# sangminwoo/Temporal-Span-Proposal-Network-VidVRD

Measured on AMD Instinct MI355X. Metric: tracklet-pairs/sec scored (N=32, T=150, D=2048), higher is better.
Workload: dtype f32

## Files before the change

### include/tspn_mi355x.h

```cpp
#ifndef TSPN_MI355X_H
#define TSPN_MI355X_H

#include <stddef.h>
#include <stdint.h>

#ifdef __cplusplus
extern "C" {
#endif

#define TSPN_ABI_VERSION 7

enum {
  TSPN_OK = 0,
  TSPN_EINVAL = -1,
  TSPN_EUNSUPPORTED = -2,
  TSPN_EWORKSPACE = -3,
  TSPN_ELAUNCH = -4,
  TSPN_EDEVICE = -5
};

#define TSPN_STATUS_WORDS 16
enum {
  TSPN_STATUS_FAULT = 0,
  TSPN_STATUS_FAULT_INFO = 1,
// ... 74 lines not shown
int tspn_conv3_f32(const float* x, int64_t B, int64_t Cin, int64_t T,
                   const float* packed, int64_t M, const float* bias, int relu,
                   float* y, void* stream);

int tspn_conv3_tc_f32(const float* x, int64_t B, int64_t T, int64_t Cin,
                      const float* packed, int64_t M, const float* bias, int relu,
                      float* y, void* stream);

int tspn_pack_conv3_wino63_frag_f32(const float* W, int64_t M, int64_t Cin, int64_t split, float* frag,
                                    void* stream);
size_t tspn_conv3_tc_wino63_workspace_bytes(int64_t B, int64_t T, int64_t Cin);
int tspn_conv3_tc_wino63_f32(const float* x, int64_t B, int64_t T, int64_t Cin, const float* frag,
                             int64_t M, const float* bias, int relu, float* y,
                             void* workspace, size_t workspace_bytes, void* stream);
int tspn_conv3_tc_wino63_set_piece_form(int form);

size_t tspn_pack_conv3_wino63_f16x3_elements(int64_t M, int64_t Cin, int64_t split);
int tspn_pack_conv3_wino63_f16x3(const float* W, int64_t M, int64_t Cin, int64_t split, int16_t* packed, void* stream);
size_t tspn_conv3_tc_wino63_f16x3_workspace_bytes(int64_t B, int64_t T, int64_t Cin, int64_t M);
int tspn_conv3_tc_wino63_f16x3(const float* x, int64_t B, int64_t T, int64_t Cin, const int16_t* packed,
                               int64_t M, const float* bias, int relu, float* y,
                               void* workspace, size_t workspace_bytes, void* stream);
int tspn_conv3_tc_wino63_f16x3_set_tail_split(int on);
int tspn_conv3_tc_wino63_f16x3_input_form(int64_t NT, int64_t T, int64_t Cin, int cus);
int tspn_conv3_tc_wino63_f16x3_set_input_form(int form);
int tspn_conv3_tc_wino63_f16x3_input(const float* x, int64_t B, int64_t T, int64_t Cin, int64_t M, void* split_input,
                                     size_t split_input_bytes, float* fbar, uint64_t* hot_slots, void* stream);


int tspn_heads_f32(int mode, const float* a, const float* b, int64_t lda,
                   const int64_t* ia, const int64_t* ib, int64_t idx_stride, const float* bias,
                   const float* Wh, const float* bh, int64_t H,
                   int64_t P, int64_t C, int64_t T, float* out, void* stream);

int tspn_heads_pairgrid_f32(const float* y, int64_t B, int64_t N, int64_t C, int64_t T,
                            const float* Wh, const float* bh, int64_t H, float* out,
                            void* stream);

size_t tspn_heads_pairgrid_f16x3_split_bytes(int64_t C, int64_t H);
int tspn_heads_pairgrid_f16x3_set_force_exact(int on);
int tspn_heads_pair_f16x3_set_diag_skip(int on);
int tspn_heads_pairgrid_f16x3(const float* y, int64_t ldt, int64_t B, int64_t N, int64_t C, int64_t T,
                              const float* Wh, const float* bh, int64_t H, void* split_buf, size_t split_bytes,
                              float* out, void* stream);

int tspn_temporal_mean_f32(const float* x, int64_t R, int64_t T, int64_t Cdim,
// ... 258 lines not shown
```

### temporal-span-proposal-network-vidvrd_amd/_abi.py

```python
import ctypes
import os
import re
import threading

HERE = os.path.dirname(os.path.abspath(__file__))
ROOT = os.path.dirname(HERE)
LIB_PATH = os.environ.get("TSPN_LIB_PATH") or os.path.join(HERE, "libtspn_mi355x.so")
HEADER_PATH = os.path.join(ROOT, "include", "tspn_mi355x.h")

ABI_VERSION = 7
TSPN_OK = 0
TSPN_EINVAL = -1
TSPN_EUNSUPPORTED = -2
TSPN_EWORKSPACE = -3
TSPN_ELAUNCH = -4
TSPN_EDEVICE = -5
STATUS_WORDS = 16
STATUS_FAULT, STATUS_FAULT_INFO, STATUS_CONV_ERR, STATUS_CONV_CHECKS = 0, 1, 2, 3
FAULT_HANDOVER = 1
CONV_CHECK_HOT_OFFSET, CONV_CHECK_SCRATCH_BYTES = 256, 256 + 256 * 64
GEOM_CHANNELS = 8
CONV_DIRECT, CONV_WINOGRAD63, CONV_WINOGRAD63_F16X3 = 0, 1, 2

_c_f32p = ctypes.c_void_p
# ... 102 lines not shown
                                               _vp, _vp]),
    "tspn_bottleneck_block_res_bf16": (_int, [_vp, _i64, _i64, _i64, _i64, _i64, _i64, _vp, _vp, _vp, _vp, _vp, _vp, _vp, _vp, _vp]),
    "tspn_bottleneck_tail_io_bf16": (_int, [_vp, _i64, _i64, _i64, _i64, _vp, _vp, _vp, _vp, _vp, _vp, _vp]),
    "tspn_bottleneck_tail_pipe_bf16": (_int, [_vp, _i64, _i64, _i64, _i64, _vp, _vp, _vp, _vp, _vp, _vp, _i64, _vp]),
    "tspn_bottleneck_tail_next_bf16": (_int, [_vp, _i64, _i64, _i64, _i64, _vp, _vp, _vp, _vp, _vp, _vp, _vp, _vp, _vp, _vp]),
    "tspn_stem_bf16_workspace_bytes": (_sz, [_i64, _i64, _i64]),
    "tspn_pack_stem_bf16": (_int, [_vp, _i64, _vp, _vp]),
    "tspn_stem_conv_bf16": (_int, [_vp, _i64, _i64, _i64, _vp, _i64, _vp, _vp, _sz, _vp, _vp]),
    "tspn_max_pool_nhwc_bf16": (_int, [_vp, _i64, _i64, _i64, _i64, _i64, _i64, _i64, _vp, _vp]),
    "tspn_stem_pool_bf16": (_int, [_vp, _i64, _i64, _i64, _vp, _i64, _vp, _vp, _sz, _vp, _vp]),
    "tspn_roi_align_nhwc_bf16": (_int, [_vp, _i64, _i64, _i64, _i64, _vp, _i64, _i64, ctypes.c_float, _int, _int,
                                        _int, _vp, _vp]),
    "tspn_roi_align_nhwc_f32_bf16out": (_int, [_vp, _i64, _i64, _i64, _i64, _vp, _i64, _i64, ctypes.c_float, _int, _int,
                                               _int, _vp, _vp]),
    "tspn_pack_conv3_wino63_frag_f32": (_int, [_vp, _i64, _i64, _i64, _vp, _vp]),
    "tspn_conv3_tc_wino63_workspace_bytes": (_sz, [_i64, _i64, _i64]),
    "tspn_conv3_tc_wino63_f32": (_int, [_vp, _i64, _i64, _i64, _vp, _i64, _vp, _int, _vp, _vp, _sz, _vp]),
    "tspn_conv3_tc_wino63_set_piece_form": (_int, [_int]),
    "tspn_pack_conv3_wino63_f16x3_elements": (_sz, [_i64, _i64, _i64]),
    "tspn_pack_conv3_wino63_f16x3": (_int, [_vp, _i64, _i64, _i64, _vp, _vp]),
    "tspn_conv3_tc_wino63_f16x3_workspace_bytes": (_sz, [_i64, _i64, _i64, _i64]),
    "tspn_conv3_tc_wino63_f16x3": (_int, [_vp, _i64, _i64, _i64, _vp, _i64, _vp, _int, _vp, _vp, _sz, _vp]),
    "tspn_conv3_tc_wino63_f16x3_set_tail_split": (_int, [_int]),
    "tspn_conv3_tc_wino63_f16x3_input_form": (_int, [_i64, _i64, _i64, _int]),
    "tspn_conv3_tc_wino63_f16x3_set_input_form": (_int, [_int]),
    "tspn_conv3_tc_wino63_f16x3_input": (_int, [_vp, _i64, _i64, _i64, _i64, _vp, _sz, _vp, _vp, _vp]),
    "tspn_span_predicate_workspace_bytes": (_sz, [_i64, _i64, _i64, _i64]),
    "tspn_span_predicate_f32": (_int, [_vp, _i64, _i64, _i64, _vp, _vp, _i64, _vp, _vp, _i64, _vp, _vp, _sz, _vp]),
    "tspn_decode_span_relations_workspace_bytes": (_sz, [_i64] * 8),
    "tspn_decode_span_relations_f32": (_int, [_vp, _i64, _i64, _i64, _i64, _vp, _i64, _vp, _vp, _vp, _i64, _vp, _vp, _i64,
                                              _vp, _i64, _i64, _i64, _vp, _vp, _vp, _vp, _vp, _vp, _vp, _sz, _vp]),
    "tspn_cast_bf16": (_int, [_vp, _i64, _vp, _vp]),
    "tspn_pack_conv3_bf16": (_int, [_vp, _i64, _i64, _i64, _vp, _vp]),
    "tspn_transpose_cast_bf16": (_int, [_vp, _i64, _i64, _i64, _vp, _vp]),
    "tspn_heads_dense_bf16": (_int, [_vp, _i64, _i64, _i64, _i64, _vp, _vp, _i64, _vp, _vp]),
    "tspn_temporal_encoder_heads_bf16": (_int, [_vp, _i64, _i64, _i64, _vp, _vp, _vp, _vp, _i64, _vp, _vp, _vp]),
    "tspn_pack_heads_bf16": (_int, [_vp, _i64, _i64, _vp, _vp]),
    "tspn_conv3_tc_bf16": (_int, [_vp, _i64, _i64, _i64, _vp, _i64, _vp, _vp, _i64, _vp]),
    "tspn_heads_pairgrid_bf16": (_int, [_vp, _i64, _i64, _i64, _i64, _i64, _vp, _vp, _i64, _vp, _vp]),
    "tspn_temporal_mean_bf16": (_int, [_vp, _i64, _i64, _i64, _vp, _vp]),
    "tspn_forward_fused_bf16_workspace_bytes": (_sz, [ctypes.POINTER(FusedBf16Desc)]),
    "tspn_forward_fused_bf16": (_int, [ctypes.POINTER(FusedBf16Desc), _vp]),
    "tspn_pair_plan_i32": (_int, [_vp, _i64, _i64, _i64, _vp, _vp, _vp, _vp, _vp, _vp, _vp]),
    "tspn_heads_pairlist_bf16_workspace_bytes": (_sz, [_i64, _i64, _i64]),
    "tspn_heads_pairlist_bf16": (_int, [_vp, _i64, _i64, _i64, _i64, _i64, _vp, _i64, _vp, _vp, _i64, _vp, _vp, _sz, _vp]),
    "tspn_forward_fused_bf16_pairs_workspace_bytes": (_sz, [ctypes.POINTER(FusedBf16Desc)]),
# ... 79 lines not shown
```

### temporal-span-proposal-network-vidvrd_amd/csrc/tspn_wino63.hip

```cpp
#include <algorithm>
#include <atomic>
#include <type_traits>

#include "tspn_common.h"
#include "tspn_device.h"
#include "tspn_wino63_input.h"

namespace {

using namespace tspn_dev;

constexpr int NW = 4;
constexpr int THREADS = 64 * NW;
constexpr int BM = 128;
constexpr int ST = 32;
constexpr int SWG = 64;
constexpr int KC = 8;
constexpr int NJ = 8;
constexpr int VROW = ST * 4;
constexpr int VCH = 2 * NJ * VROW;
constexpr int VHALF = 4 * VCH;
constexpr int VSS = 2 * VHALF;
constexpr int NVB = 2;
constexpr int NPIECE = 16;
// ... 393 lines not shown
    f32x4 V[2][8];
    transform(cg, V, false, xm);
#pragma unroll
    for (int j = 0; j < NJ; ++j) {
      f16x8 hi, lo;
#pragma unroll
      for (int i = 0; i < 8; ++i) {
        _Float16 h, l;
        wino63_split_f16(V[i >> 2][j][i & 3], ecol[j], h, l);
        hi[i] = h;
        lo[i] = l;
      }
      _Float16* dst = Vh + (((int64_t)j * 2 * ncg + cg) * nsp2 + S) * 8;
      *reinterpret_cast<f16x8*>(dst) = hi;
      *reinterpret_cast<f16x8*>(dst + (int64_t)ncg * nsp2 * 8) = lo;
    }
  }
}

#ifndef TSPN_WINO63_F16X3_STAGGER
#define TSPN_WINO63_F16X3_STAGGER 1
#endif
template <int WN, bool BUF>
__device__ __forceinline__ void wino63_f16x3_tile(
    char* smem_raw, const _Float16* __restrict__ Vh, const int* __restrict__ Ve, const int16_t* __restrict__ Wp,
    const float* __restrict__ bias, float* __restrict__ y, float* __restrict__ park, int Cin, int T, int M, int nq,
    int64_t nsext, int64_t nsp2, int tile_m, int tile_n, int tiles_n, int sub, int relu, int ldy, int vec2) {
  constexpr int MI = WN;
  constexpr int BN = 64 * WN;
  constexpr int NP = 16 + 4 * WN;
  constexpr int PW = (NP + 7) / 8;
  constexpr bool EVEN = NP % 8 == 0;
  constexpr bool STAGGER = TSPN_WINO63_F16X3_STAGGER && WN == 4;
  const int m0 = tile_m * F_BM;
  const int64_t S0 = (int64_t)tile_n * F_BN + sub * BN;

  const int tid = threadIdx.x;
  const int lane = tid & 63;
  const int wave = __builtin_amdgcn_readfirstlane(tid >> 6);
  const int wm = wave / WN, wn = wave % WN;
  const int li = lane & 31, kh = lane >> 5;
  const int ncg = Cin >> 3, nk = Cin >> 4;
  const int G = NJ * nk;

  const int p0 = wave * NP / 8;
  const int npw = EVEN ? PW : (wave + 1) * NP / 8 - p0;
  const int16_t* src[PW];
  unsigned voff[PW];
  int ldst[PW];
#pragma unroll
  for (int i = 0; i < PW; ++i) {
    const int p = min(p0 + i, NP - 1);
    int64_t el;
    if (p < 16) {
      const int region = p >> 3, cgi = (p >> 2) & 1, r = 64 * (p & 3) + lane;
      el = (((int64_t)region * ncg + cgi) * M + m0 + r) * 8;
      src[i] = Wp + el;
      ldst[i] = p * 1024;
    } else {
      const int v = p - 16;
      const int region = v / (2 * WN), cgi = (v / WN) & 1, r = 64 * (v % WN) + lane;
      el = (((int64_t)region * ncg + cgi) * nsp2 + S0 + r) * 8;
      src[i] = reinterpret_cast<const int16_t*>(Vh) + el;
      ldst[i] = (2 + region) * 8192 + cgi * 4096 + (v % WN) * 1024;
    }
    voff[i] = (unsigned)(el * 2);
  }
  int ik = 0, ist = 0;
  const char* wbase = reinterpret_cast<const char*>(Wp);
  const char* vbase = reinterpret_cast<const char*>(Vh);
  auto issue = [&]() {
    char* dst = smem_raw + ist * F_ST;
#pragma unroll
    for (int i = 0; i < PW; ++i)
      if (EVEN || i < npw) {
        if (BUF) bglds16(buffer_rsrc_unbounded(p0 + i < 16 ? wbase : vbase), voff[i], 0, dst + ldst[i]);
        else glds16(src[i], dst + ldst[i]);
      }
    ist = (ist + 1) & 3;
    const bool wrap = ++ik == nk;
    if (wrap) ik = 0;
    const int64_t dw = (int64_t)M * (wrap ? 32 * nk + 48 : 32), dv = nsp2 * (wrap ? 32 * nk + 32 : 32);
    if (BUF) {
      wbase += dw;
      vbase += dv;
    } else {
#pragma unroll
      for (int i = 0; i < PW; ++i) src[i] = reinterpret_cast<const int16_t*>(reinterpret_cast<const char*>(src[i]) + (p0 + i < 16 ? dw : dv));
    }
  };
  auto wait_stages = [&](auto ahead_tag) {
    constexpr int AHEAD = decltype(ahead_tag)::value;
    if (EVEN || npw == PW) wait_vmcnt<AHEAD * PW>(); else wait_vmcnt<AHEAD * (PW - 1)>();
  };

  f32x16 acc[MI][2];
#pragma unroll
  for (int mi = 0; mi < MI; ++mi)
#pragma unroll
    for (int ni = 0; ni < 2; ++ni)
#pragma unroll
      for (int e = 0; e < 16; ++e) acc[mi][ni][e] = 0.f;

  float* my_park = park + (int64_t)(tile_m * tiles_n + tile_n) * (F_PARK_PER_TILE / sizeof(float)) +
                   (int64_t)sub * (8 * MI) * F_THREADS * 4 + tid * 4;
  int* etab = reinterpret_cast<int*>(smem_raw + F_SMEM);
  auto unscale = [&](int j) {
    if (tid < F_BM)
      etab[tid] = reinterpret_cast<const int*>(Wp + (int64_t)j * (2 * ncg + 1) * M * 8 + (int64_t)2 * ncg * M * 8)[(int64_t)(m0 + tid) * 4];
    else if (tid - F_BM < BN)
      etab[tid] = Ve[(int64_t)j * nsp2 + S0 + tid - F_BM];
    __syncthreads();
    int ec[2];
#pragma unroll
    for (int ni = 0; ni < 2; ++ni) ec[ni] = etab[F_BM + wn * 64 + ni * 32 + li];
#pragma unroll
    for (int mi = 0; mi < MI; ++mi)
// ... 33 lines not shown
#pragma unroll
      for (int mi = 0; mi < MI; ++mi)
#pragma unroll
        for (int ni = 0; ni < 2; ++ni)
#pragma unroll
          for (int eq = 0; eq < 4; ++eq) {
            const f32x4 v = {acc[mi][ni][4 * eq], acc[mi][ni][4 * eq + 1], acc[mi][ni][4 * eq + 2], acc[mi][ni][4 * eq + 3]};
            *reinterpret_cast<f32x4*>(my_park + ((int64_t)j * 32 + (mi * 2 + ni) * 4 + eq) * F_THREADS * 4) = v;
#pragma unroll
            for (int e = 0; e < 4; ++e) acc[mi][ni][4 * eq + e] = 0.f;
          }
    }
    __builtin_amdgcn_sched_barrier(0);
  };
  auto kstep = [&](int g, f16x8 (&bc)[2], f16x8 (&bn)[2], auto steady_tag) {
    constexpr bool STEADY = decltype(steady_tag)::value;
#define TSPN_MR(NM, NR)                                \
  __builtin_amdgcn_sched_group_barrier(0x008, NM, 0);  \
  __builtin_amdgcn_sched_group_barrier(0x100, NR, 0);
    group(ah, bc);
    read_lo(g & 3);
    if (WN == 4) { TSPN_MR(1, 1) TSPN_MR(1, 1) TSPN_MR(1, 1) TSPN_MR(1, 1) TSPN_MR(1, 1) TSPN_MR(1, 1) TSPN_MR(2, 0) }
    __builtin_amdgcn_sched_barrier(0);
    if (STEADY || g + 2 < G) wait_stages(std::integral_constant<int, 1>{});
    else wait_vmcnt<0>();
    __builtin_amdgcn_s_barrier();
    __builtin_amdgcn_sched_barrier(0);
    const bool more = STEADY || g + 3 < G;
    if (more && (!STAGGER || wm == 0)) issue();
    __builtin_amdgcn_sched_barrier(0);
    group(ah, bl);
    __builtin_amdgcn_sched_barrier(0);
    if (STAGGER && more && wm != 0) issue();
    __builtin_amdgcn_sched_barrier(0);
    group(al, bc);
    if (STEADY || g + 1 < G) read_hi((g + 1) & 3, bn);
    if (WN == 4 && STEADY) { TSPN_MR(2, 1) TSPN_MR(1, 1) TSPN_MR(1, 1) TSPN_MR(1, 1) TSPN_MR(1, 1) TSPN_MR(1, 1) TSPN_MR(1, 0) }
#undef TSPN_MR
    __builtin_amdgcn_sched_barrier(0);
  };

  issue();
  issue();
  issue();
  wait_stages(std::integral_constant<int, 2>{});
  __builtin_amdgcn_s_barrier();
  __builtin_amdgcn_sched_barrier(0);
  read_hi(0, bh[0]);
  int g = 0, kc = 0, jc = 0;
  auto pair = [&](auto steady_tag) {
    kstep(g, bh[0], bh[1], steady_tag);
    kstep(g + 1, bh[1], bh[0], steady_tag);
    g += 2;
    kc += 2;
    if (kc == nk) {
      point_end(jc);
      kc = 0;
      ++jc;
    }
  };
  while (g + 4 < G) pair(std::true_type{});
  while (g < G) pair(std::false_type{});

  wait_vmcnt<0>();
#pragma unroll
  for (int ni = 0; ni < 2; ++ni) {
    const int64_t Sx = S0 + wn * 64 + ni * 32 + li;
    const bool col_ok = Sx < nsext;
    const int64_t b = col_ok ? Sx / nq : 0;
    const int q = col_ok ? (int)(Sx - b * nq) : 0;
    const int t = 6 * q;
    float* ycol = y + (b * M) * (int64_t)ldy + t;
#pragma unroll
    for (int mi = 0; mi < MI; ++mi)
#pragma unroll
      for (int eq = 0; eq < 4; ++eq) {
        f32x4 P[NJ - 1];
#pragma unroll
        for (int j = 0; j < NJ - 1; ++j)
          P[j] = *reinterpret_cast<const f32x4*>(my_park + ((int64_t)j * 32 + (mi * 2 + ni) * 4 + eq) * F_THREADS * 4);
        if (!col_ok) continue;
#pragma unroll
        for (int e4 = 0; e4 < 4; ++e4) {
          const int e = 4 * eq + e4;
          const int m = m0 + wm * (32 * MI) + mi * 32 + (e & 3) + 8 * (e >> 2) + 4 * kh;
          const float p12 = P[1][e4] + P[2][e4], m12 = P[1][e4] - P[2][e4];
          const float p34 = P[3][e4] + P[4][e4], m34 = P[3][e4] - P[4][e4];
          const float p56 = P[5][e4] + P[6][e4], m56 = P[5][e4] - P[6][e4];
          float o[6];
          o[0] = P[0][e4] + p12 + p34 + p56;
          o[1] = m12 + 2.f * m34 + 0.5f * m56;
          o[2] = p12 + 4.f * p34 + 0.25f * p56;
          o[3] = m12 + 8.f * m34 + 0.125f * m56;
          o[4] = p12 + 16.f * p34 + 0.0625f * p56;
          o[5] = m12 + 32.f * m34 + 0.03125f * m56 + acc[mi][ni][e];
          if (bias != nullptr) {
            const float bb = bias[m];
#pragma unroll
            for (int i = 0; i < 6; ++i) o[i] += bb;
          }
          if (relu) {
#pragma unroll
            for (int i = 0; i < 6; ++i) o[i] = tspn::relu_f32(o[i]);
          }
          float* dst = ycol + (int64_t)m * ldy;
          if (vec2) {
            *reinterpret_cast<f32x2*>(dst) = f32x2{o[0], o[1]};
            *reinterpret_cast<f32x2*>(dst + 2) = f32x2{o[2], o[3]};
            *reinterpret_cast<f32x2*>(dst + 4) = f32x2{o[4], o[5]};
          } else {
#pragma unroll
            for (int i = 0; i < 6; ++i)
              if (t + i < T) dst[i] = o[i];
          }
        }
      }
  }
}

__global__ __launch_bounds__(F_THREADS, 1) void conv3_wino63_kernel(
    const _Float16* __restrict__ Vh, const int* __restrict__ Ve, const int16_t* __restrict__ Wp,
    const float* __restrict__ bias, float* __restrict__ y, float* __restrict__ park, int Cin, int T, int M, int nq,
    int64_t nsext, int64_t nsp2, int tiles_m, int tiles_n, int relu, int ldy, int GM, int vec2) {
  extern __shared__ __attribute__((aligned(16))) char smem_raw[];

  const int f = max((GM >> 8) & 0xff, 1);
  const bool buf = (GM >> 16) & 1;
  GM &= 0xff;
  const int tiles = tiles_m * tiles_n;
  const int nsplit = f > 1 ? ((int)gridDim.x - tiles) / (f - 1) : 0;
  const int nfull = tiles - nsplit;
  const int bid = blockIdx.x;
  int wg, sub = 0;
  if (bid < nfull) {
    wg = xcd_remap(bid, nfull);
  } else {
    const int s = xcd_remap(bid - nfull, nsplit * f);
    wg = nfull + s / f;
    sub = s - (s / f) * f;
  }
  int tile_m, tile_n;
  grouped_tile(wg, GM, tiles_m, tiles_n, tile_m, tile_n);
  auto tile = [&](auto wn_tag, auto buf_tag) {
    wino63_f16x3_tile<decltype(wn_tag)::value, decltype(buf_tag)::value>(
        smem_raw, Vh, Ve, Wp, bias, y, park, Cin, T, M, nq, nsext, nsp2, tile_m, tile_n, tiles_n, sub, relu, ldy, vec2);
  };
  auto shape = [&](auto buf_tag) {
    if (bid < nfull) tile(std::integral_constant<int, 4>{}, buf_tag);
    else if (f == 2) tile(std::integral_constant<int, 2>{}, buf_tag);
    else tile(std::integral_constant<int, 1>{}, buf_tag);
  };
  if (buf) shape(std::true_type{}); else shape(std::false_type{});
}

int64_t padded_sextets(int64_t B, int64_t T) { return tspn::ceil_div(B * tspn::ceil_div(T, 6), SWG) * SWG; }
int64_t padded_sextets_f16x3(int64_t B, int64_t T) { return tspn::ceil_div(B * tspn::ceil_div(T, 6), F_BN) * F_BN; }

struct F16x3Layout {
  size_t v, e, park, total;
};
F16x3Layout f16x3_layout(int64_t B, int64_t T, int64_t Cin, int64_t M) {
  F16x3Layout L{};
  const size_t nsp2 = (size_t)padded_sextets_f16x3(B, T);
  L.v = 0;
  L.e = tspn::align_up((size_t)NJ * 2 * Cin * nsp2 * sizeof(_Float16), 256);
  L.park = L.e + tspn::align_up((size_t)NJ * nsp2 * sizeof(int), 256);
  L.total = L.park + (size_t)tspn::ceil_div(M, F_BM) * (nsp2 / F_BN) * F_PARK_PER_TILE;
  return L;
// ... 159 lines not shown
               workspace_bytes, L.total);
  TSPN_REQUIRE((reinterpret_cast<uintptr_t>(workspace) & 255) == 0, TSPN_EINVAL, "%s: workspace must be 256-byte aligned",
               what);
  const int64_t nq = tspn::ceil_div(T, 6);
  const int64_t nsext = B * nq, nsp2 = padded_sextets_f16x3(B, T);
  TSPN_REQUIRE(nsp2 / 8 < (1LL << 31), TSPN_EUNSUPPORTED, "%s: grid too large", what);
  char* ws = static_cast<char*>(workspace);
  if (fused_in)
    return tspn::input_f16x3(x, B, T, Cin, nsp2, reinterpret_cast<_Float16*>(ws + L.v), reinterpret_cast<int*>(ws + L.e), fbar,
                             hot, stream, stages);
  void (*kern)(const float*, _Float16*, int*, int, int, int, int64_t, int64_t, int64_t, unsigned long long*) =
      wino63_input_transform_kernel;
  hipLaunchKernelGGL(kern, dim3((unsigned)(nsp2 / 8)), dim3(256), 0, TSPN_STREAM(stream), x,
                     reinterpret_cast<_Float16*>(ws + L.v), reinterpret_cast<int*>(ws + L.e), (int)T, (int)Cin, (int)nq,
                     nsext, nsp2, B * T, reinterpret_cast<unsigned long long*>(hot));
  return tspn::check_launch(what);
}

static std::atomic<int> g_tail_split{1};

extern "C" int tspn_conv3_tc_wino63_f16x3_set_tail_split(int on) {
  TSPN_REQUIRE(on == 0 || on == 1, TSPN_EINVAL, "tspn_conv3_tc_wino63_f16x3_set_tail_split: on must be 0 or 1");
  return g_tail_split.exchange(on, std::memory_order_relaxed);
}

static int device_cus() {
  constexpr int kMaxDevices = 64;
  static std::atomic<int> cached[kMaxDevices] = {};
  int dev = -1, cus = 0;
  if (hipGetDevice(&dev) != hipSuccess) return 0;
  const bool tracked = dev >= 0 && dev < kMaxDevices;
  if (tracked && (cus = cached[dev].load(std::memory_order_relaxed)) > 0) return cus;
  if (hipDeviceGetAttribute(&cus, hipDeviceAttributeMultiprocessorCount, dev) != hipSuccess || cus <= 0) return 0;
  if (tracked) cached[dev].store(cus, std::memory_order_relaxed);
  return cus;
}

extern "C" int tspn_conv3_tc_wino63_f16x3_input_form(int64_t NT, int64_t T, int64_t Cin, int cus) {
  if (NT <= 0 || cus <= 0 || !tspn::input_f16x3_supported(T, Cin)) return 0;
  return Cin >= 1024 && 2 * NT >= cus;
}

static std::atomic<int> g_input_form{0};

extern "C" int tspn_conv3_tc_wino63_f16x3_set_input_form(int form) {
  TSPN_REQUIRE(form >= 0 && form <= 2, TSPN_EINVAL, "tspn_conv3_tc_wino63_f16x3_set_input_form: form must be 0, 1 or 2");
// ... 30 lines not shown
  TSPN_REQUIRE(tspn::aligned16(packed) && (reinterpret_cast<uintptr_t>(y) & 3) == 0,
               TSPN_EUNSUPPORTED, "%s: packed weights must be 16-byte aligned", what);
  const F16x3Layout L = f16x3_layout(B, T, Cin, M);
  TSPN_REQUIRE(workspace_bytes >= L.total, TSPN_EWORKSPACE, "%s: workspace %zu < %zu bytes", what, workspace_bytes,
               L.total);
  const int64_t nq = tspn::ceil_div(T, 6);
  const int64_t nsext = B * nq, nsp2 = padded_sextets_f16x3(B, T);
  const int64_t tiles_m = M / F_BM, tiles_n = nsp2 / F_BN;
  TSPN_REQUIRE(tiles_m * tiles_n < (1LL << 29), TSPN_EUNSUPPORTED, "%s: grid too large", what);
  const int vec2 = (ldy % 2 == 0) && (ldy >= 6 * nq) && ((reinterpret_cast<uintptr_t>(y) & 7) == 0);
  int64_t R = 0;
  const int f = tail_split_factor(tiles_m * tiles_n, device_cus(), &R);
  const int64_t grid = tiles_m * tiles_n + R * (f - 1);
  const int64_t slab = 4 * Cin * std::max<int64_t>(M, nsp2);
  const int buf = slab < (1LL << 31) && g_piece_form.load(std::memory_order_relaxed) == 0;
  char* ws = static_cast<char*>(workspace);
  static tspn::LdsLimit lds;
  void (*kern)(const _Float16*, const int*, const int16_t*, const float*, float*, float*, int, int, int, int, int64_t,
               int64_t, int, int, int, int, int, int) = conv3_wino63_kernel;
  if (int rc = lds.ensure(reinterpret_cast<const void*>(kern), F_SMEM_ALL, what)) return rc;
  hipLaunchKernelGGL(kern, dim3((unsigned)grid), dim3(F_THREADS), F_SMEM_ALL, TSPN_STREAM(stream),
                     reinterpret_cast<const _Float16*>(ws + L.v), reinterpret_cast<const int*>(ws + L.e), packed, bias, y,
                     reinterpret_cast<float*>(ws + L.park), (int)Cin, (int)T, (int)M, (int)nq, nsext, nsp2, (int)tiles_m,
                     (int)tiles_n, relu, (int)ldy, TSPN_WINO63_GM | (f << 8) | (buf << 16), vec2);
  return tspn::check_launch(what);
}

extern "C" int tspn_conv3_tc_wino63_f16x3(const float* x, int64_t B, int64_t T, int64_t Cin, const int16_t* packed,
                                          int64_t M, const float* bias, int relu, float* y, void* workspace,
                                          size_t workspace_bytes, void* stream) {
  const char* what = "tspn_conv3_tc_wino63_f16x3";
  if (int rc = check_common(what, B, T, Cin, M, T)) return rc;
  TSPN_REQUIRE(tspn::wino63_f16x3_supported(Cin, M), TSPN_EUNSUPPORTED,
               "%s: needs Cin %% 32 == 0 and M %% 256 == 0 (Cin=%lld M=%lld)", what, (long long)Cin, (long long)M);
  if (B > 0) {
    TSPN_REQUIRE(workspace && packed && y, TSPN_EINVAL, "%s: null pointer", what);
    TSPN_REQUIRE(tspn::aligned16(packed) && (reinterpret_cast<uintptr_t>(y) & 3) == 0,
                 TSPN_EUNSUPPORTED, "%s: packed weights must be 16-byte aligned", what);
  }
  if (int rc = tspn::wino63_f16x3_input_transform(x, B, T, Cin, M, workspace, workspace_bytes, stream, nullptr,
                                                  tspn::wino63_f16x3_fused_input(B, T, Cin)))
    return rc;
  return tspn::wino63_f16x3_contract(workspace, workspace_bytes, B, T, Cin, packed, M, bias, relu, y, T, stream);
}

extern "C" int tspn_conv3_tc_wino63_f16x3_input(const float* x, int64_t B, int64_t T, int64_t Cin, int64_t M, void* split_input,
                                                size_t split_input_bytes, float* fbar, uint64_t* hot_slots, void* stream) {
// ... 9 lines not shown
```

### temporal-span-proposal-network-vidvrd_amd/ops.py

```python
import ctypes
import threading

import torch

from . import _abi

__all__ = [
    "predicate_head", "feature_preprocess_", "ppn_pair_matrix_topk", "traj_iou", "traj_iou_tail", "pair_index",
    "pair_gather", "pack_conv3", "conv3", "conv3_tc", "pack_conv3_wino63", "conv3_tc_wino63", "pack_conv3_wino63_f16x3", "conv3_tc_wino63_f16x3", "heads", "heads_pairgrid", "heads_pairgrid_f16x3", "heads_pairgrid_f16x3_split_bytes",
    "heads_pairgrid_f16x3_set_force_exact", "heads_pair_f16x3_set_diag_skip","temporal_mean", "temporal_sum", "pair_rows", "transpose_td",
    "forward_fused", "temporal_encoder_heads", "fused_workspace_bytes", "fused_bf16_workspace_bytes", "decode_topk", "decode_spans", "decode_span_relations",
    "span_anchor_labels", "span_loss", "span_anchor_sample", "pair_labels", "span_match",
    "cast_bf16", "pack_conv3_bf16", "pack_heads_bf16", "conv3_tc_bf16", "heads_pairgrid_bf16",
    "pair_plan", "heads_pairlist_bf16",
    "transpose_cast_bf16", "temporal_encoder_heads_bf16",
    "temporal_mean_bf16", "forward_fused_bf16", "span_predicate",
    "pack_span_cls_bf16", "span_predicate_bf16", "decode_span_relations_bf16", "bottleneck_block_bf16", "bottleneck_block_proj_bf16", "bottleneck_block_res_bf16",
    "proposal_pair_filter", "gather_rows", "wino63_set_piece_form", "wino63_f16x3_set_tail_split", "conv3_spot_check",
    "wino63_f16x3_set_input_form", "wino63_f16x3_input_form", "wino63_f16x3_input",
    "pack_conv2d", "pack_conv2d_frag", "conv2d_nhwc", "roi_align_nhwc", "pack_conv2d_frag_bf16", "conv2d_nhwc_bf16", "max_pool_nhwc", "pack_conv2d_frag_cin4", "conv2d_nhwc_cin4", "max_pool_nhwc_bf16", "pack_stem_bf16", "stem_conv_bf16", "stem_pool_bf16", "bottleneck_tail_bf16",
    "eval_traj_volume", "eval_viou", "eval_greedy_match", "evalobj_tiou", "evalobj_claim",
    "status_words", "status_fault", "status_clear", "status_selftest",
]


_status_blocks = {}
_status_lock = threading.Lock()


def _status_block(index=None):
    idx = torch.cuda.current_device() if index is None else int(index)
    blk = _status_blocks.get(idx)
    if blk is not None:
        return blk
    with _status_lock:
        blk = _status_blocks.get(idx)
        if blk is None:
            raw = torch.zeros(_abi.STATUS_WORDS + 16, dtype=torch.int32).pin_memory()
            off = (-(raw.data_ptr() // 4)) % 16
            blk = raw[off:off + _abi.STATUS_WORDS]
            with torch.cuda.device(idx):
# ... 406 lines not shown
def conv3_tc_wino63_f16x3(x, packed, bias=None, relu=False, workspace=None):
    _dev(x, "x")
    if bias is not None:
        _dev(bias, "bias")
    B, T, Cin = x.shape
    cin_w, M = wino63_f16x3_dims(packed)
    if cin_w != Cin:
        raise ValueError(f"conv3_tc_wino63_f16x3: weights are for Cin={cin_w}, x has Cin={Cin}")
    l = _abi.lib()
    need = l.tspn_conv3_tc_wino63_f16x3_workspace_bytes(B, T, Cin, M)
    workspace = _workspace(workspace, need, x.device, "conv3_tc_wino63_f16x3", sizes=True)
    y = torch.empty((B, M, T), dtype=torch.float32, device=x.device)
    _abi.check(l.tspn_conv3_tc_wino63_f16x3(_p(x), B, T, Cin, _p(packed), M, _p(bias), 1 if relu else 0, _p(y),
                                            _p(workspace), workspace.numel() * workspace.element_size(), _stream()))
    return y


def wino63_set_piece_form(form):
    return _toggle("tspn_conv3_tc_wino63_set_piece_form", form)


def wino63_f16x3_set_tail_split(on):
    return _toggle("tspn_conv3_tc_wino63_f16x3_set_tail_split", on)


def wino63_f16x3_set_input_form(form):
    return _toggle("tspn_conv3_tc_wino63_f16x3_set_input_form", form)


def wino63_f16x3_input_form(NT, T, Cin, cus):
    return int(_abi.lib().tspn_conv3_tc_wino63_f16x3_input_form(int(NT), int(T), int(Cin), int(cus)))


def wino63_f16x3_input(x, M, workspace=None, mean=True, hot=True):
    _dev(x, "x")
    B, T, Cin = x.shape
    l = _abi.lib()
    need = l.tspn_conv3_tc_wino63_f16x3_workspace_bytes(B, T, Cin, M)
    workspace = _workspace(workspace, need, x.device, "wino63_f16x3_input", sizes=True)
    fbar = torch.empty((B, Cin), dtype=torch.float32, device=x.device) if mean else None
    slots = torch.zeros((64, 32), dtype=torch.int64, device=x.device) if hot else None
    _abi.check(l.tspn_conv3_tc_wino63_f16x3_input(_p(x), B, T, Cin, M, _p(workspace),
                                                  workspace.numel() * workspace.element_size(), _p(fbar), _p(slots), _stream()))
    nsp2 = -(-(B * (-(-T // 6))) // 256) * 256
    vbytes = 8 * 2 * Cin * nsp2 * 2
    v = workspace[:vbytes].view(torch.int16).view(8, 2, Cin // 8, nsp2, 8)
# ... 1214 lines not shown
```

Measured before the change: 1.274 million.

## Add 16x16x32 MFMA variant of the f16x3 Winograd conv tile and default to it

Adds a new tile routine for the f16x3 Winograd F(6,3) conv that uses 16x16x32 f16 MFMA instructions in place of the 32x32 shape. It has its own K-step schedule: two ring stages are issued per step, LDS reads are double-buffered and interleaved with MFMAs, and the accumulator layout and parking are reworked. The shared load ring and output transform are factored into helpers, and a runtime toggle selects the shape, defaulting to the new 16x16 path. The aim is better MFMA throughput or issue overlap on MI355X, at the cost of more LDS reads per FLOP and a more complex schedule.

```diff
diff --git a/include/tspn_mi355x.h b/include/tspn_mi355x.h
--- a/include/tspn_mi355x.h
+++ b/include/tspn_mi355x.h
@@ -120,6 +120,7 @@
                                int64_t M, const float* bias, int relu, float* y,
                                void* workspace, size_t workspace_bytes, void* stream);
 int tspn_conv3_tc_wino63_f16x3_set_tail_split(int on);
+int tspn_conv3_tc_wino63_f16x3_set_mfma_shape(int shape);
 int tspn_conv3_tc_wino63_f16x3_input_form(int64_t NT, int64_t T, int64_t Cin, int cus);
 int tspn_conv3_tc_wino63_f16x3_set_input_form(int form);
 int tspn_conv3_tc_wino63_f16x3_input(const float* x, int64_t B, int64_t T, int64_t Cin, int64_t M, void* split_input,
diff --git a/temporal-span-proposal-network-vidvrd_amd/_abi.py b/temporal-span-proposal-network-vidvrd_amd/_abi.py
--- a/temporal-span-proposal-network-vidvrd_amd/_abi.py
+++ b/temporal-span-proposal-network-vidvrd_amd/_abi.py
@@ -148,6 +148,7 @@
     "tspn_conv3_tc_wino63_f16x3_workspace_bytes": (_sz, [_i64, _i64, _i64, _i64]),
     "tspn_conv3_tc_wino63_f16x3": (_int, [_vp, _i64, _i64, _i64, _vp, _i64, _vp, _int, _vp, _vp, _sz, _vp]),
     "tspn_conv3_tc_wino63_f16x3_set_tail_split": (_int, [_int]),
+    "tspn_conv3_tc_wino63_f16x3_set_mfma_shape": (_int, [_int]),
     "tspn_conv3_tc_wino63_f16x3_input_form": (_int, [_i64, _i64, _i64, _int]),
     "tspn_conv3_tc_wino63_f16x3_set_input_form": (_int, [_int]),
     "tspn_conv3_tc_wino63_f16x3_input": (_int, [_vp, _i64, _i64, _i64, _i64, _vp, _sz, _vp, _vp, _vp]),
diff --git a/temporal-span-proposal-network-vidvrd_amd/csrc/tspn_wino63.hip b/temporal-span-proposal-network-vidvrd_amd/csrc/tspn_wino63.hip
--- a/temporal-span-proposal-network-vidvrd_amd/csrc/tspn_wino63.hip
+++ b/temporal-span-proposal-network-vidvrd_amd/csrc/tspn_wino63.hip
@@ -439,55 +439,48 @@
 #define TSPN_WINO63_F16X3_STAGGER 1
 #endif
 template <int WN, bool BUF>
-__device__ __forceinline__ void wino63_f16x3_tile(
-    char* smem_raw, const _Float16* __restrict__ Vh, const int* __restrict__ Ve, const int16_t* __restrict__ Wp,
-    const float* __restrict__ bias, float* __restrict__ y, float* __restrict__ park, int Cin, int T, int M, int nq,
-    int64_t nsext, int64_t nsp2, int tile_m, int tile_n, int tiles_n, int sub, int relu, int ldy, int vec2) {
-  constexpr int MI = WN;
-  constexpr int BN = 64 * WN;
-  constexpr int NP = 16 + 4 * WN;
-  constexpr int PW = (NP + 7) / 8;
-  constexpr bool EVEN = NP % 8 == 0;
-  constexpr bool STAGGER = TSPN_WINO63_F16X3_STAGGER && WN == 4;
-  const int m0 = tile_m * F_BM;
-  const int64_t S0 = (int64_t)tile_n * F_BN + sub * BN;
-
-  const int tid = threadIdx.x;
-  const int lane = tid & 63;
-  const int wave = __builtin_amdgcn_readfirstlane(tid >> 6);
-  const int wm = wave / WN, wn = wave % WN;
-  const int li = lane & 31, kh = lane >> 5;
-  const int ncg = Cin >> 3, nk = Cin >> 4;
-  const int G = NJ * nk;
-
-  const int p0 = wave * NP / 8;
-  const int npw = EVEN ? PW : (wave + 1) * NP / 8 - p0;
+struct F16x3Ring {
+  static constexpr int NP = 16 + 4 * WN;
+  static constexpr int PW = (NP + 7) / 8;
+  static constexpr bool EVEN = NP % 8 == 0;
+  char* smem;
+  int p0, npw;
   const int16_t* src[PW];
   unsigned voff[PW];
   int ldst[PW];
-#pragma unroll
-  for (int i = 0; i < PW; ++i) {
-    const int p = min(p0 + i, NP - 1);
-    int64_t el;
-    if (p < 16) {
-      const int region = p >> 3, cgi = (p >> 2) & 1, r = 64 * (p & 3) + lane;
-      el = (((int64_t)region * ncg + cgi) * M + m0 + r) * 8;
-      src[i] = Wp + el;
-      ldst[i] = p * 1024;
-    } else {
-      const int v = p - 16;
-      const int region = v / (2 * WN), cgi = (v / WN) & 1, r = 64 * (v % WN) + lane;
-      el = (((int64_t)region * ncg + cgi) * nsp2 + S0 + r) * 8;
-      src[i] = reinterpret_cast<const int16_t*>(Vh) + el;
-      ldst[i] = (2 + region) * 8192 + cgi * 4096 + (v % WN) * 1024;
-    }
-    voff[i] = (unsigned)(el * 2);
-  }
-  int ik = 0, ist = 0;
-  const char* wbase = reinterpret_cast<const char*>(Wp);
-  const char* vbase = reinterpret_cast<const char*>(Vh);
-  auto issue = [&]() {
-    char* dst = smem_raw + ist * F_ST;
+  int ik = 0, ist = 0, nk, M;
+  int64_t nsp2;
+  const char* wbase;
+  const char* vbase;
+
+  __device__ __forceinline__ F16x3Ring(char* smem_raw, const _Float16* __restrict__ Vh, const int16_t* __restrict__ Wp,
+                                       int Cin, int M_, int64_t nsp2_, int m0, int64_t S0, int wave, int lane)
+      : smem(smem_raw), nk(Cin >> 4), M(M_), nsp2(nsp2_), wbase(reinterpret_cast<const char*>(Wp)),
+        vbase(reinterpret_cast<const char*>(Vh)) {
+    const int ncg = Cin >> 3;
+    p0 = wave * NP / 8;
+    npw = EVEN ? PW : (wave + 1) * NP / 8 - p0;
+#pragma unroll
+    for (int i = 0; i < PW; ++i) {
+      const int p = min(p0 + i, NP - 1);
+      int64_t el;
+      if (p < 16) {
+        const int region = p >> 3, cgi = (p >> 2) & 1, r = 64 * (p & 3) + lane;
+        el = (((int64_t)region * ncg + cgi) * M + m0 + r) * 8;
+        src[i] = Wp + el;
+        ldst[i] = p * 1024;
+      } else {
+        const int v = p - 16;
+        const int region = v / (2 * WN), cgi = (v / WN) & 1, r = 64 * (v % WN) + lane;
+        el = (((int64_t)region * ncg + cgi) * nsp2 + S0 + r) * 8;
+        src[i] = reinterpret_cast<const int16_t*>(Vh) + el;
+        ldst[i] = (2 + region) * 8192 + cgi * 4096 + (v % WN) * 1024;
+      }
+      voff[i] = (unsigned)(el * 2);
+    }
+  }
+  __device__ __forceinline__ void issue() {
+    char* dst = smem + ist * F_ST;
 #pragma unroll
     for (int i = 0; i < PW; ++i)
       if (EVEN || i < npw) {
@@ -505,11 +498,64 @@
 #pragma unroll
       for (int i = 0; i < PW; ++i) src[i] = reinterpret_cast<const int16_t*>(reinterpret_cast<const char*>(src[i]) + (p0 + i < 16 ? dw : dv));
     }
-  };
-  auto wait_stages = [&](auto ahead_tag) {
-    constexpr int AHEAD = decltype(ahead_tag)::value;
+  }
+  template <int AHEAD>
+  __device__ __forceinline__ void wait_stages() const {
     if (EVEN || npw == PW) wait_vmcnt<AHEAD * PW>(); else wait_vmcnt<AHEAD * (PW - 1)>();
-  };
+  }
+};
+
+__device__ __forceinline__ void wino63_f16x3_store(const f32x4 (&P)[NJ - 1], int e4, float a7, const float* __restrict__ bias,
+                                                   int m, int relu, float* __restrict__ dst, int vec2, int t, int T) {
+  const float p12 = P[1][e4] + P[2][e4], m12 = P[1][e4] - P[2][e4];
+  const float p34 = P[3][e4] + P[4][e4], m34 = P[3][e4] - P[4][e4];
+  const float p56 = P[5][e4] + P[6][e4], m56 = P[5][e4] - P[6][e4];
+  float o[6];
+  o[0] = P[0][e4] + p12 + p34 + p56;
+  o[1] = m12 + 2.f * m34 + 0.5f * m56;
+  o[2] = p12 + 4.f * p34 + 0.25f * p56;
+  o[3] = m12 + 8.f * m34 + 0.125f * m56;
+  o[4] = p12 + 16.f * p34 + 0.0625f * p56;
+  o[5] = m12 + 32.f * m34 + 0.03125f * m56 + a7;
+  if (bias != nullptr) {
+    const float bb = bias[m];
+#pragma unroll
+    for (int i = 0; i < 6; ++i) o[i] += bb;
+  }
+  if (relu) {
+#pragma unroll
+    for (int i = 0; i < 6; ++i) o[i] = tspn::relu_f32(o[i]);
+  }
+  if (vec2) {
+    *reinterpret_cast<f32x2*>(dst) = f32x2{o[0], o[1]};
+    *reinterpret_cast<f32x2*>(dst + 2) = f32x2{o[2], o[3]};
+    *reinterpret_cast<f32x2*>(dst + 4) = f32x2{o[4], o[5]};
+  } else {
+#pragma unroll
+    for (int i = 0; i < 6; ++i)
+      if (t + i < T) dst[i] = o[i];
+  }
+}
+
+template <int WN, bool BUF>
+__device__ __forceinline__ void wino63_f16x3_tile(
+    char* smem_raw, const _Float16* __restrict__ Vh, const int* __restrict__ Ve, const int16_t* __restrict__ Wp,
+    const float* __restrict__ bias, float* __restrict__ y, float* __restrict__ park, int Cin, int T, int M, int nq,
+    int64_t nsext, int64_t nsp2, int tile_m, int tile_n, int tiles_n, int sub, int relu, int ldy, int vec2) {
+  constexpr int MI = WN;
+  constexpr int BN = 64 * WN;
+  constexpr bool STAGGER = TSPN_WINO63_F16X3_STAGGER && WN == 4;
+  const int m0 = tile_m * F_BM;
+  const int64_t S0 = (int64_t)tile_n * F_BN + sub * BN;
+
+  const int tid = threadIdx.x;
+  const int lane = tid & 63;
+  const int wave = __builtin_amdgcn_readfirstlane(tid >> 6);
+  const int wm = wave / WN, wn = wave % WN;
+  const int li = lane & 31, kh = lane >> 5;
+  const int ncg = Cin >> 3, nk = Cin >> 4;
+  const int G = NJ * nk;
+  F16x3Ring<WN, BUF> ring(smem_raw, Vh, Wp, Cin, M, nsp2, m0, S0, wave, lane);
 
   f32x16 acc[MI][2];
 #pragma unroll
@@ -589,16 +635,16 @@
     read_lo(g & 3);
     if (WN == 4) { TSPN_MR(1, 1) TSPN_MR(1, 1) TSPN_MR(1, 1) TSPN_MR(1, 1) TSPN_MR(1, 1) TSPN_MR(1, 1) TSPN_MR(2, 0) }
     __builtin_amdgcn_sched_barrier(0);
-    if (STEADY || g + 2 < G) wait_stages(std::integral_constant<int, 1>{});
+    if (STEADY || g + 2 < G) ring.template wait_stages<1>();
     else wait_vmcnt<0>();
     __builtin_amdgcn_s_barrier();
     __builtin_amdgcn_sched_barrier(0);
     const bool more = STEADY || g + 3 < G;
-    if (more && (!STAGGER || wm == 0)) issue();
+    if (more && (!STAGGER || wm == 0)) ring.issue();
     __builtin_amdgcn_sched_barrier(0);
     group(ah, bl);
     __builtin_amdgcn_sched_barrier(0);
-    if (STAGGER && more && wm != 0) issue();
+    if (STAGGER && more && wm != 0) ring.issue();
     __builtin_amdgcn_sched_barrier(0);
     group(al, bc);
     if (STEADY || g + 1 < G) read_hi((g + 1) & 3, bn);
@@ -607,10 +653,10 @@
     __builtin_amdgcn_sched_barrier(0);
   };
 
-  issue();
-  issue();
-  issue();
-  wait_stages(std::integral_constant<int, 2>{});
+  ring.issue();
+  ring.issue();
+  ring.issue();
+  ring.template wait_stages<2>();
   __builtin_amdgcn_s_barrier();
   __builtin_amdgcn_sched_barrier(0);
   read_hi(0, bh[0]);
@@ -651,37 +697,187 @@
         for (int e4 = 0; e4 < 4; ++e4) {
           const int e = 4 * eq + e4;
           const int m = m0 + wm * (32 * MI) + mi * 32 + (e & 3) + 8 * (e >> 2) + 4 * kh;
-          const float p12 = P[1][e4] + P[2][e4], m12 = P[1][e4] - P[2][e4];
-          const float p34 = P[3][e4] + P[4][e4], m34 = P[3][e4] - P[4][e4];
-          const float p56 = P[5][e4] + P[6][e4], m56 = P[5][e4] - P[6][e4];
-          float o[6];
-          o[0] = P[0][e4] + p12 + p34 + p56;
-          o[1] = m12 + 2.f * m34 + 0.5f * m56;
-          o[2] = p12 + 4.f * p34 + 0.25f * p56;
-          o[3] = m12 + 8.f * m34 + 0.125f * m56;
-          o[4] = p12 + 16.f * p34 + 0.0625f * p56;
-          o[5] = m12 + 32.f * m34 + 0.03125f * m56 + acc[mi][ni][e];
-          if (bias != nullptr) {
-            const float bb = bias[m];
-#pragma unroll
-            for (int i = 0; i < 6; ++i) o[i] += bb;
-          }
-          if (relu) {
-#pragma unroll
-            for (int i = 0; i < 6; ++i) o[i] = tspn::relu_f32(o[i]);
-          }
-          float* dst = ycol + (int64_t)m * ldy;
-          if (vec2) {
-            *reinterpret_cast<f32x2*>(dst) = f32x2{o[0], o[1]};
-            *reinterpret_cast<f32x2*>(dst + 2) = f32x2{o[2], o[3]};
-            *reinterpret_cast<f32x2*>(dst + 4) = f32x2{o[4], o[5]};
-          } else {
-#pragma unroll
-            for (int i = 0; i < 6; ++i)
-              if (t + i < T) dst[i] = o[i];
-          }
+          wino63_f16x3_store(P, e4, acc[mi][ni][e], bias, m, relu, ycol + (int64_t)m * ldy, vec2, t, T);
         }
       }
+  }
+}
+
+template <int WN, bool BUF>
+__device__ __forceinline__ void wino63_f16x3_tile16(
+    char* smem_raw, const _Float16* __restrict__ Vh, const int* __restrict__ Ve, const int16_t* __restrict__ Wp,
+    const float* __restrict__ bias, float* __restrict__ y, float* __restrict__ park, int Cin, int T, int M, int nq,
+    int64_t nsext, int64_t nsp2, int tile_m, int tile_n, int tiles_n, int sub, int relu, int ldy, int vec2) {
+  constexpr int NB = 2 * WN;
+  constexpr int BN = 64 * WN;
+  constexpr bool STAGGER = TSPN_WINO63_F16X3_STAGGER && WN == 4;
+  const int m0 = tile_m * F_BM;
+  const int64_t S0 = (int64_t)tile_n * F_BN + sub * BN;
+
+  const int tid = threadIdx.x;
+  const int lane = tid & 63;
+  const int wave = __builtin_amdgcn_readfirstlane(tid >> 6);
+  const int wm = wave / WN, wn = wave % WN;
+  const int l16 = lane & 15, kq = lane >> 4;
+  const int ncg = Cin >> 3, nss = Cin >> 5;
+  const int G = NJ * nss;
+  F16x3Ring<WN, BUF> ring(smem_raw, Vh, Wp, Cin, M, nsp2, m0, S0, wave, lane);
+
+  f32x4 acc[NB][4];
+#pragma unroll
+  for (int bi = 0; bi < NB; ++bi)
+#pragma unroll
+    for (int bj = 0; bj < 4; ++bj) acc[bi][bj] = f32x4{0.f, 0.f, 0.f, 0.f};
+
+  float* my_park = park + (int64_t)(tile_m * tiles_n + tile_n) * (F_PARK_PER_TILE / sizeof(float)) +
+                   (int64_t)sub * (4 * NB) * F_THREADS * 4 + tid * 4;
+  int* etab = reinterpret_cast<int*>(smem_raw + F_SMEM);
+  auto unscale = [&](int j) {
+    if (tid < F_BM)
+      etab[tid] = reinterpret_cast<const int*>(Wp + (int64_t)j * (2 * ncg + 1) * M * 8 + (int64_t)2 * ncg * M * 8)[(int64_t)(m0 + tid) * 4];
+    else if (tid - F_BM < BN)
+      etab[tid] = Ve[(int64_t)j * nsp2 + S0 + tid - F_BM];
+    __syncthreads();
+    int ec[4];
+#pragma unroll
+    for (int bj = 0; bj < 4; ++bj) ec[bj] = etab[F_BM + wn * 64 + bj * 16 + l16];
+#pragma unroll
+    for (int bi = 0; bi < NB; ++bi)
+#pragma unroll
+      for (int e = 0; e < 4; ++e) {
+        const int r = etab[wm * (16 * NB) + bi * 16 + 4 * kq + e];
+#pragma unroll
+        for (int bj = 0; bj < 4; ++bj) acc[bi][bj][e] = ldexpf(acc[bi][bj][e], -(r + ec[bj]));
+      }
+  };
+
+  f16x8 ah[2], al[2], bh[4], bl[4];
+  const int k_off = (kq >> 1) * F_ST + (kq & 1) * 4096;
+  const int a_off = k_off + (wm * (16 * NB) + l16) * 16, b_off = k_off + 16384 + (wn * 64 + l16) * 16;
+  auto read_a = [&](int s, int bi, int buffer) {
+    const char* p = smem_raw + (s & 1) * (2 * F_ST) + a_off + bi * 256;
+    ah[buffer] = *reinterpret_cast<const f16x8*>(p);
+    al[buffer] = *reinterpret_cast<const f16x8*>(p + 8192);
+  };
+  auto read_b = [&](int s, int lo, f16x8 (&b)[4]) {
+    const char* p = smem_raw + (s & 1) * (2 * F_ST) + b_off + lo * 8192;
+#pragma unroll
+    for (int bj = 0; bj < 4; ++bj) b[bj] = *reinterpret_cast<const f16x8*>(p + bj * 256);
+  };
+  auto group = [&](int bi, const f16x8& a, const f16x8 (&b)[4]) {
+#pragma unroll
+    for (int bj = 0; bj < 4; ++bj) acc[bi][bj] = __builtin_amdgcn_mfma_f32_16x16x32_f16(a, b[bj], acc[bi][bj], 0, 0, 0);
+  };
+  auto point_end = [&](int j) {
+    unscale(j);
+    if (j < NJ - 1) {
+#pragma unroll
+      for (int bi = 0; bi < NB; ++bi)
+#pragma unroll
+        for (int bj = 0; bj < 4; ++bj) {
+          *reinterpret_cast<f32x4*>(my_park + ((int64_t)j * 32 + bi * 4 + bj) * F_THREADS * 4) = acc[bi][bj];
+          acc[bi][bj] = f32x4{0.f, 0.f, 0.f, 0.f};
+        }
+    }
+    __builtin_amdgcn_sched_barrier(0);
+  };
+  auto sstep = [&](int s, auto steady_tag) {
+    constexpr bool STEADY = decltype(steady_tag)::value;
+#define TSPN_MR(NM, NR)                                \
+  __builtin_amdgcn_sched_group_barrier(0x008, NM, 0);  \
+  __builtin_amdgcn_sched_group_barrier(0x100, NR, 0);
+#pragma unroll
+    for (int bi = 0; bi < NB - 1; ++bi) {
+      if (STAGGER && bi == 0 && wm != 0 && s > 0 && STEADY) {
+        ring.issue();
+        ring.issue();
+        __builtin_amdgcn_sched_barrier(0);
+      }
+      group(bi, ah[bi & 1], bh);
+      read_a(s, bi + 1, (bi + 1) & 1);
+      group(bi, ah[bi & 1], bl);
+      group(bi, al[bi & 1], bh);
+      TSPN_MR(2, 1) TSPN_MR(2, 1) TSPN_MR(8, 0)
+      __builtin_amdgcn_sched_barrier(0);
+    }
+    constexpr int bi = NB - 1;
+    asm volatile("s_waitcnt lgkmcnt(0)" ::: "memory");
+    if (STEADY) wait_vmcnt<0>();
+    __builtin_amdgcn_s_barrier();
+    __builtin_amdgcn_sched_barrier(0);
+    if (STEADY && s + 2 < G && (!STAGGER || wm == 0)) {
+      ring.issue();
+      ring.issue();
+      __builtin_amdgcn_sched_barrier(0);
+    }
+    group(bi, ah[bi & 1], bh);
+    if (STEADY) {
+      read_a(s + 1, 0, 0);
+      TSPN_MR(2, 1) TSPN_MR(2, 1)
+    }
+    __builtin_amdgcn_sched_barrier(0);
+#pragma unroll
+    for (int bj = 0; bj < 4; ++bj) {
+      acc[bi][bj] = __builtin_amdgcn_mfma_f32_16x16x32_f16(ah[bi & 1], bl[bj], acc[bi][bj], 0, 0, 0);
+      if (STEADY) bl[bj] = *reinterpret_cast<const f16x8*>(smem_raw + ((s + 1) & 1) * (2 * F_ST) + b_off + 8192 + bj * 256);
+    }
+    if (STEADY) { TSPN_MR(1, 1) TSPN_MR(1, 1) TSPN_MR(1, 1) TSPN_MR(1, 1) }
+    __builtin_amdgcn_sched_barrier(0);
+#pragma unroll
+    for (int bj = 0; bj < 4; ++bj) {
+      acc[bi][bj] = __builtin_amdgcn_mfma_f32_16x16x32_f16(al[bi & 1], bh[bj], acc[bi][bj], 0, 0, 0);
+      if (STEADY) bh[bj] = *reinterpret_cast<const f16x8*>(smem_raw + ((s + 1) & 1) * (2 * F_ST) + b_off + bj * 256);
+    }
+    if (STEADY) { TSPN_MR(1, 1) TSPN_MR(1, 1) TSPN_MR(1, 1) TSPN_MR(1, 1) }
+#undef TSPN_MR
+    __builtin_amdgcn_sched_barrier(0);
+  };
+
+  ring.issue();
+  ring.issue();
+  ring.issue();
+  ring.issue();
+  ring.template wait_stages<2>();
+  __builtin_amdgcn_s_barrier();
+  __builtin_amdgcn_sched_barrier(0);
+  read_b(0, 0, bh);
+  read_b(0, 1, bl);
+  read_a(0, 0, 0);
+  int s = 0, kc = 0, jc = 0;
+  auto step = [&](auto steady_tag) {
+    sstep(s, steady_tag);
+    ++s;
+    if (++kc == nss) {
+      point_end(jc);
+      kc = 0;
+      ++jc;
+    }
+  };
+  while (s + 1 < G) step(std::true_type{});
+  step(std::false_type{});
+
+  wait_vmcnt<0>();
+#pragma unroll
+  for (int bj = 0; bj < 4; ++bj) {
+    const int64_t Sx = S0 + wn * 64 + bj * 16 + l16;
+    const bool col_ok = Sx < nsext;
+    const int64_t b = col_ok ? Sx / nq : 0;
+    const int q = col_ok ? (int)(Sx - b * nq) : 0;
+    const int t = 6 * q;
+    float* ycol = y + (b * M) * (int64_t)ldy + t;
+#pragma unroll
+    for (int bi = 0; bi < NB; ++bi) {
+      f32x4 P[NJ - 1];
+#pragma unroll
+      for (int j = 0; j < NJ - 1; ++j)
+        P[j] = *reinterpret_cast<const f32x4*>(my_park + ((int64_t)j * 32 + bi * 4 + bj) * F_THREADS * 4);
+      if (!col_ok) continue;
+#pragma unroll
+      for (int e = 0; e < 4; ++e) {
+        const int m = m0 + wm * (16 * NB) + bi * 16 + 4 * kq + e;
+        wino63_f16x3_store(P, e, acc[bi][bj][e], bias, m, relu, ycol + (int64_t)m * ldy, vec2, t, T);
+      }
+    }
   }
 }
 
@@ -693,6 +889,7 @@
 
   const int f = max((GM >> 8) & 0xff, 1);
   const bool buf = (GM >> 16) & 1;
+  const bool s16 = (GM >> 17) & 1;
   GM &= 0xff;
   const int tiles = tiles_m * tiles_n;
   const int nsplit = f > 1 ? ((int)gridDim.x - tiles) / (f - 1) : 0;
@@ -709,8 +906,12 @@
   int tile_m, tile_n;
   grouped_tile(wg, GM, tiles_m, tiles_n, tile_m, tile_n);
   auto tile = [&](auto wn_tag, auto buf_tag) {
-    wino63_f16x3_tile<decltype(wn_tag)::value, decltype(buf_tag)::value>(
-        smem_raw, Vh, Ve, Wp, bias, y, park, Cin, T, M, nq, nsext, nsp2, tile_m, tile_n, tiles_n, sub, relu, ldy, vec2);
+    if (s16)
+      wino63_f16x3_tile16<decltype(wn_tag)::value, decltype(buf_tag)::value>(
+          smem_raw, Vh, Ve, Wp, bias, y, park, Cin, T, M, nq, nsext, nsp2, tile_m, tile_n, tiles_n, sub, relu, ldy, vec2);
+    else
+      wino63_f16x3_tile<decltype(wn_tag)::value, decltype(buf_tag)::value>(
+          smem_raw, Vh, Ve, Wp, bias, y, park, Cin, T, M, nq, nsext, nsp2, tile_m, tile_n, tiles_n, sub, relu, ldy, vec2);
   };
   auto shape = [&](auto buf_tag) {
     if (bid < nfull) tile(std::integral_constant<int, 4>{}, buf_tag);
@@ -916,6 +1117,13 @@
 extern "C" int tspn_conv3_tc_wino63_f16x3_set_tail_split(int on) {
   TSPN_REQUIRE(on == 0 || on == 1, TSPN_EINVAL, "tspn_conv3_tc_wino63_f16x3_set_tail_split: on must be 0 or 1");
   return g_tail_split.exchange(on, std::memory_order_relaxed);
+}
+
+static std::atomic<int> g_mfma_shape{1};
+
+extern "C" int tspn_conv3_tc_wino63_f16x3_set_mfma_shape(int shape) {
+  TSPN_REQUIRE(shape == 0 || shape == 1, TSPN_EINVAL, "tspn_conv3_tc_wino63_f16x3_set_mfma_shape: shape must be 0 or 1");
+  return g_mfma_shape.exchange(shape, std::memory_order_relaxed);
 }
 
 static int device_cus() {
@@ -992,7 +1200,8 @@
   hipLaunchKernelGGL(kern, dim3((unsigned)grid), dim3(F_THREADS), F_SMEM_ALL, TSPN_STREAM(stream),
                      reinterpret_cast<const _Float16*>(ws + L.v), reinterpret_cast<const int*>(ws + L.e), packed, bias, y,
                      reinterpret_cast<float*>(ws + L.park), (int)Cin, (int)T, (int)M, (int)nq, nsext, nsp2, (int)tiles_m,
-                     (int)tiles_n, relu, (int)ldy, TSPN_WINO63_GM | (f << 8) | (buf << 16), vec2);
+                     (int)tiles_n, relu, (int)ldy,
+                     TSPN_WINO63_GM | (f << 8) | (buf << 16) | (g_mfma_shape.load(std::memory_order_relaxed) << 17), vec2);
   return tspn::check_launch(what);
 }
 
diff --git a/temporal-span-proposal-network-vidvrd_amd/ops.py b/temporal-span-proposal-network-vidvrd_amd/ops.py
--- a/temporal-span-proposal-network-vidvrd_amd/ops.py
+++ b/temporal-span-proposal-network-vidvrd_amd/ops.py
@@ -16,7 +16,7 @@
     "transpose_cast_bf16", "temporal_encoder_heads_bf16",
     "temporal_mean_bf16", "forward_fused_bf16", "span_predicate",
     "pack_span_cls_bf16", "span_predicate_bf16", "decode_span_relations_bf16", "bottleneck_block_bf16", "bottleneck_block_proj_bf16", "bottleneck_block_res_bf16",
-    "proposal_pair_filter", "gather_rows", "wino63_set_piece_form", "wino63_f16x3_set_tail_split", "conv3_spot_check",
+    "proposal_pair_filter", "gather_rows", "wino63_set_piece_form", "wino63_f16x3_set_tail_split", "wino63_f16x3_set_mfma_shape", "conv3_spot_check",
     "wino63_f16x3_set_input_form", "wino63_f16x3_input_form", "wino63_f16x3_input",
     "pack_conv2d", "pack_conv2d_frag", "conv2d_nhwc", "roi_align_nhwc", "pack_conv2d_frag_bf16", "conv2d_nhwc_bf16", "max_pool_nhwc", "pack_conv2d_frag_cin4", "conv2d_nhwc_cin4", "max_pool_nhwc_bf16", "pack_stem_bf16", "stem_conv_bf16", "stem_pool_bf16", "bottleneck_tail_bf16",
     "eval_traj_volume", "eval_viou", "eval_greedy_match", "evalobj_tiou", "evalobj_claim",
@@ -469,6 +469,10 @@
 
 def wino63_f16x3_set_tail_split(on):
     return _toggle("tspn_conv3_tc_wino63_f16x3_set_tail_split", on)
+
+
+def wino63_f16x3_set_mfma_shape(shape):
+    return _toggle("tspn_conv3_tc_wino63_f16x3_set_mfma_shape", shape)
 
 
 def wino63_f16x3_set_input_form(form):
```

New measurement: 1.173 million. 0.921x the previous value.
